# hzyu17/GaussianVI

Measured on AMD Instinct MI355X. Metric: sigma-point psi-evals/sec + NGD iters/sec, 1024-factor d=12 p=5 chain, higher is better.
Workload: dtype f64; 1 GPU; c3: T=1025 states, n=6; 1 step = 1 device-resident NGD iteration; restart every 30; factor_sets_columns=[K factors, d, GH degree p, N sigma points], factor_set_kinds=1024 x quadratic-prior d=12 p=5 (N=17217); 1025 x fixed-prior d=6 p=5 (N=1433), kernel_variant=6, chunks_per_factor=4, fused_pass=True, one_launch_factor_stage=False, mirror_pairs=False, fuse_trial=2

## Files before the change

### gaussianvi_amd/csrc/gvi_hip.hip

```cpp
#include "../../include/gvi_hip.h"

#include <hip/hip_runtime.h>
#include <hip/hip_ext.h>
#include <dlfcn.h>

#include <algorithm>
#include <chrono>
#include <cassert>
#include <cmath>
#include <cstdio>
#include <cstdlib>
#include <cstring>
#include <memory>
#include <map>
#include <set>
#include <string>
#include <thread>
#include <vector>

#include "host_linalg.hpp"
#include "kernels_bt.hpp"
#include "chain_launch.hpp"
#include "kernels_factor.hpp"
#include "kernels_orbit.hpp"
// ... 516 lines not shown
  }
  if (s.kind == KIND_QUAD_PRIOR) {
    switch (d) {
      case 2: launch_reg<2, PsiQuad<2, 1>>(a, grid, st); return true;
      case 4: launch_reg<4, PsiQuad<4, 2>>(a, grid, st); return true;
      case 6: launch_reg<6, PsiQuad<6, 3>>(a, grid, st); return true;
      case 8: launch_reg<8, PsiQuad<8, 4>>(a, grid, st); return true;
      case 12: launch_reg<12, PsiQuad<12, 6>>(a, grid, st); return true;
    }
  }
  if (s.kind == KIND_FIXED_PRIOR) {
    switch (d) {
      case 1: launch_reg<1, PsiQuad<1, 1>>(a, grid, st); return true;
      case 2: launch_reg<2, PsiQuad<2, 2>>(a, grid, st); return true;
      case 3: launch_reg<3, PsiQuad<3, 3>>(a, grid, st); return true;
      case 4: launch_reg<4, PsiQuad<4, 4>>(a, grid, st); return true;
      case 6: launch_reg<6, PsiQuad<6, 6>>(a, grid, st); return true;
      case 8: launch_reg<8, PsiQuad<8, 8>>(a, grid, st); return true;
      case 12: launch_reg<12, PsiQuad<12, 12>>(a, grid, st); return true;
    }
  }
  return false;
}

void dispatch_scost(gvi_ctx* c, const FactorSet& s, const MomArgs& a, int nchunk, hipStream_t st) {
  launch_scost<2>(s, a, nchunk, st);
}

bool orbit_supported(const gvi_ctx* c, const FactorSet& s) {
  if (!c->orbit || !(c->variant == 0 || c->variant == 6)) return false;
  if (s.kind != KIND_QUAD_PRIOR && s.kind != KIND_FIXED_PRIOR) return false;
  if (!(s.m == 2 || s.m == 6 || s.m == 12 || (s.m == 14 && s.table->orb.smax <= 4)) || s.d > 32) return false;
  if (s.m == 2 && s.table->orb.smax > 4) return false;
  const OrbitHost& o = s.table->orb;
  return o.ok && o.smax >= 1 && o.smax <= ORBIT_SMAX && !o.tile_s.empty();
}

gvi_status orbit_args(gvi_ctx* c, FactorSet& s, int full, OrbitArgs* out) {
  Table& t = *s.table;
  auto it = t.orb_bounds.find(s.nchunk);
  if (it == t.orb_bounds.end()) {
    const std::vector<int32_t> b = orbit_chunk_bounds(t.orb, s.nchunk);
    auto mem = std::make_unique<DevMem>();
    HIPCK(c, mem->ensure(b.size() * 4));
    HIPCK(c, hipMemcpy(mem->p, b.data(), b.size() * 4, hipMemcpyHostToDevice));
    it = t.orb_bounds.emplace(s.nchunk, std::move(mem)).first;
  }
  OrbitArgs a;
  a.H = s.H.d(); a.u0 = s.u0.d(); a.sgn = s.sgn.d(); a.partial = s.partial.d();
  a.K = s.K; a.d = s.d; a.nchunk = s.nchunk;
  a.pred = c->cur_pred; a.pred_val = c->cur_pred_val;
  const int waves = ((s.m == 6 && t.orb.smax <= 4) || s.m == 2) ? 4 : ((s.m == 12 && t.orb.smax <= 4) ? 3 : 2);
  const size_t lds_cap = std::min<size_t>(64 * 1024, 160 * 1024 / waves);
  a.copies = 1;
  while (a.copies * 2 <= c->orbit_copies && (size_t)4 * orbit_lds_doubles(s.d, s.m, a.copies * 2) * 8 <= lds_cap) a.copies *= 2;
  a.ob.cpk = (const uint64_t*)t.orb_cpk.p; a.ob.rpk = (const uint64_t*)t.orb_rpk.p; a.ob.mag = t.orb_mag.d(); a.ob.w = t.orb_w.d();
  a.ob.bounds = it->second->i();
  a.ob.norb_p = t.orb.norb_p; a.ob.w0 = t.orb.w0;
  {
    int32_t cum = 0;
    for (int sz = 7; sz >= 0; --sz) {
      if (sz >= 1 && sz <= t.orb.smax) cum += t.orb.cstride[sz] / 64;
      a.ob.cend[sz] = sz > t.orb.smax ? 0 : cum;
    }
    for (int sz = 0; sz < 8; ++sz) {
      const bool in = sz >= 1 && sz <= t.orb.smax;
      a.ob.cbase[sz] = in ? t.orb.cbase[sz] : 0;
      a.ob.cgrp[sz] = in ? t.orb.cgrp[sz] : 1;
      a.ob.cstride[sz] = in ? t.orb.cstride[sz] : 0;
    }
    a.ob.nb = 0;
    for (int i = 0; i < 5; ++i) a.ob.bnd[i] = 0;
    if (s.nchunk <= 4) {
      const std::vector<int32_t> b = orbit_chunk_bounds(t.orb, s.nchunk);
      a.ob.nb = s.nchunk;
      for (int i = 0; i <= s.nchunk; ++i) a.ob.bnd[i] = b[(size_t)i];
    }
  }
  (void)full;
  *out = a;
  return GVI_OK;
}

template <int M, int SMAX, int WAVES>
void launch_orbit_t(const OrbitArgs& a, bool full, bool all_pos, dim3 grid, size_t lds, hipStream_t st) {
  if (full && all_pos) hipLaunchKernelGGL((moments_orbit_kernel<M, SMAX, true, false, WAVES>), grid, dim3(256), lds, st, a);
  else if (full) hipLaunchKernelGGL((moments_orbit_kernel<M, SMAX, true, true, WAVES>), grid, dim3(256), lds, st, a);
  else if (all_pos) hipLaunchKernelGGL((moments_orbit_kernel<M, SMAX, false, false, WAVES>), grid, dim3(256), lds, st, a);
  else hipLaunchKernelGGL((moments_orbit_kernel<M, SMAX, false, true, WAVES>), grid, dim3(256), lds, st, a);
}

void launch_orbit(const OrbitArgs& a, int m, int smax, bool full, bool all_pos, hipStream_t st) {
  const dim3 grid((a.K + 3) / 4, a.nchunk);
  const size_t lds = (size_t)4 * orbit_lds_doubles(a.d, m, a.copies) * 8;
  if (m == 2) launch_orbit_t<2, 4, 4>(a, full, all_pos, grid, lds, st);
  else if (m == 14) launch_orbit_t<14, 4, 2>(a, full, all_pos, grid, lds, st);
  else if (m == 6 && smax <= 4) launch_orbit_t<6, 4, 4>(a, full, all_pos, grid, lds, st);
  else if (m == 6) launch_orbit_t<6, 6, 2>(a, full, all_pos, grid, lds, st);
  else if (smax <= 4) launch_orbit_t<12, 4, 3>(a, full, all_pos, grid, lds, st);
  else launch_orbit_t<12, 6, 2>(a, full, all_pos, grid, lds, st);
}

template <int M, int SMAX, int WAVES>
void launch_orbit_pair_t(const OrbitArgs& a0, const OrbitArgs& a1, bool full, size_t lds, hipStream_t st, hipEvent_t e0, hipEvent_t e1,
                         bool stack) {
  const int nbx0 = (a0.K + 3) / 4, nbx1 = (a1.K + 3) / 4;
  const int nb0 = nbx0 * a0.nchunk, nb1 = nbx1 * a1.nchunk;
  const int grid = stack ? std::max(nb0, nb1) : nb0 + nb1;
// ... 2840 lines not shown
```

### gaussianvi_amd/csrc/kernels_orbit.hpp

```cpp
#pragma once
#include <hip/hip_runtime.h>
#include <stdint.h>

#include "kernels_factor.hpp"

namespace gvi {

#ifdef GVI_FUSED_TIMING
__device__ unsigned long long* gvi_walk_stamps;
#endif

struct OrbitDev {
  const uint64_t* cpk;
  const uint64_t* rpk;
  const double* mag;
  const double* w;
  const int32_t* bounds;
  int64_t norb_p;
  double w0;
  int32_t cend[8];
  int32_t bnd[5];
  int32_t nb;
  int32_t cbase[8], cgrp[8], cstride[8];
};

template <int S>
struct OrbitRec { uint64_t cpk, rpk; double w; double mg[S]; };
template <typename T>
__device__ __forceinline__ T orbit_ld(const T* base, const uint32_t boff) { return *(const T*)((const char*)base + boff); }
template <int S>
__device__ __forceinline__ void orbit_load(const OrbitDev& ob, const uint32_t boff, OrbitRec<S>& r) {
  r.cpk = orbit_ld(ob.cpk, boff);
  if constexpr (S >= 1) r.rpk = orbit_ld(ob.rpk, boff);
  r.w = orbit_ld(ob.w, boff);
#pragma unroll
  for (int j = 0; j < S; ++j) r.mg[j] = orbit_ld(ob.mag + (size_t)j * ob.norb_p, boff);
}
struct OrbitNoPre { __device__ __forceinline__ void operator()() const {} };

template <int CTRL>
__device__ __forceinline__ double dpp_f64(const double v) {
  const int lo = __builtin_amdgcn_update_dpp(0, __double2loint(v), CTRL, 0xf, 0xf, false);
  const int hi = __builtin_amdgcn_update_dpp(0, __double2hiint(v), CTRL, 0xf, 0xf, false);
  return __hiloint2double(hi, lo);
}
__device__ __forceinline__ double wave_sum_f64(double v) {
  v += dpp_f64<0xB1>(v);
  v += dpp_f64<0x4E>(v);
  v += dpp_f64<0x124>(v);
  v += dpp_f64<0x128>(v);
  auto row = [&](int l) {
    return __hiloint2double(__builtin_amdgcn_readlane(__double2hiint(v), l), __builtin_amdgcn_readlane(__double2loint(v), l));
  };
  return (row(0) + row(16)) + (row(32) + row(48));
}

struct OrbitArgs {
  const double* H;
  const double* u0;
  const double* sgn;
  double* partial;
  int K, d, nchunk;
  int copies;
  const double* pred;
  double pred_val;
  OrbitDev ob;
};

__host__ __device__ constexpr int orbit_hstride(int M) { return M == 12 ? 14 : M; }

__device__ __forceinline__ void lds_add_f64(double* p, double v) {
  __hip_atomic_fetch_add(p, v, __ATOMIC_RELAXED, __HIP_MEMORY_SCOPE_WORKGROUP);
}
template <int S, typename Pre>
__device__ __forceinline__ void orbit_accumulate(const int sh, const int (&c)[S], const uint64_t rpk, const double (&mg)[S], const double wp,
                                                 const double E0, const double (&Eij)[S * (S - 1) / 2 + 1], const double (&Oi)[S],
                                                 double* accb, Pre&& pre) {
  constexpr int NV = 2 * S + S * (S - 1) / 2;
  const double w4 = wp + wp;
  double val[NV];
  {
    double mgl[S];
#pragma unroll
    for (int j = 0; j < S; ++j) { mgl[j] = mg[j]; asm volatile("" : "+v"(mgl[j]) : "v"(E0)); }
    int n = 0, e = 0;
#pragma unroll
    for (int i = 0; i < S; ++i) {
      const double wm = wp * mgl[i];
      val[n++] = w4 * mgl[i] * Oi[i];
      val[n++] = wm * mgl[i] * E0;
#pragma unroll
      for (int j = i + 1; j < S; ++j) val[n++] = wm * mgl[j] * Eij[e++];
    }
  }
  pre();
  char* const base = (char*)accb;
  char* const base1 = base + (1u << sh);
  unsigned A[S], B[S];
#pragma unroll
  for (int i = 0; i < S; ++i) {
    const unsigned lo = (unsigned)rpk, hi = (unsigned)(rpk >> 32);
    const unsigned R = i < 3 ? (lo >> (10 * i)) & 1023u : (hi >> (10 * (i - 3))) & 1023u;
    A[i] = R << sh;
    B[i] = (unsigned)c[i] << sh;
  }
  int n = 0;
#pragma unroll
  for (int i = 0; i < S; ++i) {
    lds_add_f64((double*)(base1 + B[i]), val[n]); ++n;
    lds_add_f64((double*)(base + (A[i] + B[i])), val[n]); ++n;
#pragma unroll
    for (int j = i + 1; j < S; ++j) { lds_add_f64((double*)(base + (A[i] + B[j])), val[n]); ++n; }
  }
}

template <int M, int S, bool FULL, bool SIGNED, typename Pre>
__device__ __forceinline__ void orbit_walk(const int lc, const uint64_t cpk, const uint64_t rpk, const double (&mg)[S], const double w,
                                           const double* Hl, double* accl, const double (&su0)[M], const double (&sg)[M],
                                           const double k0, double& m0, Pre&& pre) {
  int c[S];
#pragma unroll
  for (int j = 0; j < S; ++j) c[j] = (int)((cpk >> (8 * j)) & 255u);
  constexpr bool HREG = M * S <= 36 && !(M == 6 && S >= 4);
  constexpr int NH = 1 << (S - 1);
  double hcol[HREG ? S : 1][M];
  const double* hp[S];
#pragma unroll
  for (int j = 0; j < S; ++j) {
    hp[j] = Hl + c[j] * orbit_hstride(M);
    if constexpr (HREG) {
#pragma unroll
      for (int r = 0; r < M; ++r) hcol[j][r] = hp[j][r];
    }
  }
  int sig[S];
#pragma unroll
  for (int j = 0; j < S; ++j) sig[j] = j == S - 1 ? 1 : -1;
  double v[M];
#pragma unroll
  for (int r = 0; r < M; ++r) v[r] = mg[S - 1] * (HREG ? hcol[S - 1][r] : hp[S - 1][r]);
#pragma unroll
  for (int j = 0; j < S - 1; ++j) {
    if constexpr (!HREG) {
#pragma unroll
      for (int r = 0; r < M; ++r) asm volatile("" : "+v"(v[r]) :: "memory");
    }
#pragma unroll
    for (int r = 0; r < M; ++r) v[r] = fma(-mg[j], HREG ? hcol[j][r] : hp[j][r], v[r]);
  }
  constexpr bool H0REG = !HREG && M * (S + 9) <= 168;
  double h0[H0REG ? M : 1];
  if constexpr (H0REG) {
#pragma unroll
    for (int r = 0; r < M; ++r) h0[r] = hp[0][r];
  }
  constexpr bool WHT_BIG = M <= 6;
  constexpr bool WHT = FULL && S >= 2 && (S <= 4 || WHT_BIG);
  constexpr int LBMAX = S == 4 ? 2 : 3;
  constexpr int LB = S - 1 < LBMAX ? S - 1 : LBMAX;
  constexpr int BLK = 1 << LB;
  double cpv[WHT ? BLK : 1], lv[WHT ? BLK : 1];
  double E0 = 0.0, Eij[S * (S - 1) / 2 + 1], Oi[S];
#pragma unroll
  for (int e = 0; e < S * (S - 1) / 2 + 1; ++e) Eij[e] = 0.0;
#pragma unroll
  for (int j = 0; j < S; ++j) Oi[j] = 0.0;
#pragma unroll
  for (int g = 0; g < NH; ++g) {
    const int jn = g + 1 < NH ? __builtin_ctz(g + 1) : 0;
    double hn[M];
    if constexpr (!HREG) {
// ... 21 lines not shown
      if ((g & (BLK - 1)) == BLK - 1) {
#pragma unroll
        for (int j = 0; j < LB; ++j) {
#pragma unroll
          for (int bb = 0; bb < BLK; ++bb) {
            if (!(bb & (1 << j))) {
              const double c0v = cpv[bb], c1v = cpv[bb | (1 << j)], l0v = lv[bb], l1v = lv[bb | (1 << j)];
              cpv[bb] = c0v + c1v; cpv[bb | (1 << j)] = c1v - c0v;
              lv[bb] = l0v + l1v; lv[bb | (1 << j)] = l1v - l0v;
            }
          }
        }
        const bool first = g == BLK - 1;
        E0 = first ? cpv[0] : E0 + cpv[0];
        int e = 0;
#pragma unroll
        for (int i = 0; i < S; ++i) {
          {
            const double t = i < LB ? lv[1 << i] : lv[0];
            const bool pos = i < LB || sig[i] > 0;
            Oi[i] = first ? (pos ? t : -t) : (pos ? Oi[i] + t : Oi[i] - t);
          }
#pragma unroll
          for (int j = i + 1; j < S; ++j) {
            const double t = j < LB ? cpv[(1 << i) | (1 << j)] : (i < LB ? cpv[1 << i] : cpv[0]);
            const bool pos = (j < LB ? 1 : sig[j]) * (i < LB ? 1 : sig[i]) > 0;
            Eij[e] = first ? (pos ? t : -t) : (pos ? Eij[e] + t : Eij[e] - t);
            ++e;
          }
        }
      }
    } else {
      E0 += cp;
      if (FULL) {
        int e = 0;
#pragma unroll
        for (int i = 0; i < S; ++i) {
          Oi[i] = sig[i] > 0 ? Oi[i] + l : Oi[i] - l;
#pragma unroll
          for (int j = i + 1; j < S; ++j) { Eij[e] = sig[i] * sig[j] > 0 ? Eij[e] + cp : Eij[e] - cp; ++e; }
        }
      }
    }
    if (g + 1 < NH) {
      sig[jn] = -sig[jn];
      const double t2 = (sig[jn] > 0 ? 2.0 : -2.0) * mg[jn];
#pragma unroll
      for (int r = 0; r < M; ++r) v[r] = fma(t2, HREG ? hcol[jn][r] : ((H0REG && jn == 0) ? h0[r] : hn[r]), v[r]);
    }
  }
  const double wp = w + w;
  m0 = fma(wp, E0, m0);
  if constexpr (FULL) {
    orbit_accumulate<S>(lc + 3, c, rpk, mg, wp, E0, Eij, Oi, accl, pre);
  } else {
    pre();
  }
}

template <int S, bool SIGNED, typename Pre>
__device__ __forceinline__ void orbit_walk_split(const int lc, const uint64_t cpk, const uint64_t rpk, const double (&mg)[S], const double w,
                                                 const double* Hl, double* accl, const double (&su0)[12], const double (&sg)[12],
                                                 const double k0, double& m0, Pre&& pre) {
  constexpr int MH = 6, HS = orbit_hstride(12), NH = 1 << (S - 1), LB = 3, BLK = 8;
  static_assert(S >= 4 && S <= 6, "split walk: s = 4, 5, 6 (blocks of 8 Gray steps)");
  int c[S];
#pragma unroll
  for (int j = 0; j < S; ++j) c[j] = (int)((cpk >> (8 * j)) & 255u);
  double E0 = 0.0, Eij[S * (S - 1) / 2 + 1], Oi[S];
#pragma unroll
  for (int e = 0; e < S * (S - 1) / 2 + 1; ++e) Eij[e] = 0.0;
#pragma unroll
  for (int j = 0; j < S; ++j) Oi[j] = 0.0;
#pragma clang loop unroll(disable)
  for (int half = 0; half < 2; ++half) {
    double suh[MH], sgh[MH];
#pragma unroll
    for (int r = 0; r < MH; ++r) {
      suh[r] = half ? su0[MH + r] : su0[r];
      sgh[r] = SIGNED ? (half ? sg[MH + r] : sg[r]) : 1.0;
    }
    const double kk = half ? 0.0 : k0;
    double hcol[S][MH];
#pragma unroll
    for (int j = 0; j < S; ++j) {
      const double* hp = Hl + c[j] * HS + half * MH;
#pragma unroll
      for (int r = 0; r < MH; ++r) hcol[j][r] = hp[r];
    }
    int sig[S];
#pragma unroll
    for (int j = 0; j < S; ++j) sig[j] = j == S - 1 ? 1 : -1;
    double v[MH];
#pragma unroll
    for (int r = 0; r < MH; ++r) v[r] = mg[S - 1] * hcol[S - 1][r];
#pragma unroll
    for (int j = 0; j < S - 1; ++j) {
#pragma unroll
      for (int r = 0; r < MH; ++r) v[r] = fma(-mg[j], hcol[j][r], v[r]);
    }
    double cpv[BLK], lv[BLK];
#pragma unroll
    for (int g = 0; g < NH; ++g) {
      const int jn = g + 1 < NH ? __builtin_ctz(g + 1) : 0;
      double q = 0.0, l = 0.0;
#pragma unroll
      for (int r = 0; r < MH; ++r) {
        q = SIGNED ? fma(sgh[r] * v[r], v[r], q) : fma(v[r], v[r], q);
        l = fma(suh[r], v[r], l);
      }
      const double cp = q + kk;
      int b = 0;
#pragma unroll
      for (int j = 0; j < LB; ++j) b |= (sig[j] > 0 ? 1 : 0) << j;
      cpv[b] = cp;
      lv[b] = l;
      if ((g & (BLK - 1)) == BLK - 1) {
#pragma unroll
        for (int j = 0; j < LB; ++j) {
#pragma unroll
          for (int bb = 0; bb < BLK; ++bb) {
            if (!(bb & (1 << j))) {
              const double c0v = cpv[bb], c1v = cpv[bb | (1 << j)], l0v = lv[bb], l1v = lv[bb | (1 << j)];
              cpv[bb] = c0v + c1v; cpv[bb | (1 << j)] = c1v - c0v;
              lv[bb] = l0v + l1v; lv[bb | (1 << j)] = l1v - l0v;
            }
          }
        }
        E0 += cpv[0];
        int e = 0;
#pragma unroll
        for (int i = 0; i < S; ++i) {
          {
            const double t = i < LB ? lv[1 << i] : lv[0];
            const bool pos = i < LB || sig[i] > 0;
            Oi[i] = pos ? Oi[i] + t : Oi[i] - t;
          }
#pragma unroll
          for (int j = i + 1; j < S; ++j) {
            const double t = j < LB ? cpv[(1 << i) | (1 << j)] : (i < LB ? cpv[1 << i] : cpv[0]);
            const bool pos = (j < LB ? 1 : sig[j]) * (i < LB ? 1 : sig[i]) > 0;
            Eij[e] = pos ? Eij[e] + t : Eij[e] - t;
            ++e;
          }
        }
      }
      if (g + 1 < NH) {
        sig[jn] = -sig[jn];
        const double t2 = (sig[jn] > 0 ? 2.0 : -2.0) * mg[jn];
#pragma unroll
        for (int r = 0; r < MH; ++r) v[r] = fma(t2, hcol[jn][r], v[r]);
      }
    }
  }
  const double wp = w + w;
  m0 = fma(wp, E0, m0);
  orbit_accumulate<S>(lc + 3, c, rpk, mg, wp, E0, Eij, Oi, accl, pre);
}

template <int M, int S, bool FULL, bool SIGNED>
__device__ __forceinline__ void orbit_gray(const double (&hcol)[S][M], const double (&mg)[S], const double (&su0)[M], const double (&sg)[M],
                                           const double k0, double& E0, double (&Eij)[S * (S - 1) / 2 + 1], double (&Oi)[S]) {
  static_assert(S <= 3, "orbit_gray: one butterfly block");
  constexpr int NH = 1 << (S - 1), LB = S - 1, BLK = NH;
  constexpr bool WHT = FULL && S >= 2;
  int sig[S];
#pragma unroll
  for (int j = 0; j < S; ++j) sig[j] = j == S - 1 ? 1 : -1;
  double v[M];
#pragma unroll
  for (int r = 0; r < M; ++r) v[r] = mg[S - 1] * hcol[S - 1][r];
#pragma unroll
  for (int j = 0; j < S - 1; ++j) {
#pragma unroll
    for (int r = 0; r < M; ++r) v[r] = fma(-mg[j], hcol[j][r], v[r]);
  }
  double cpv[WHT ? BLK : 1], lv[WHT ? BLK : 1];
  E0 = 0.0;
#pragma unroll
  for (int e = 0; e < S * (S - 1) / 2 + 1; ++e) Eij[e] = 0.0;
#pragma unroll
  for (int j = 0; j < S; ++j) Oi[j] = 0.0;
#pragma unroll
  for (int g = 0; g < NH; ++g) {
    const int jn = g + 1 < NH ? __builtin_ctz(g + 1) : 0;
    double q = 0.0, l = 0.0;
#pragma unroll
    for (int r = 0; r < M; ++r) {
      q = SIGNED ? fma(sg[r] * v[r], v[r], q) : fma(v[r], v[r], q);
      if (FULL) l = fma(su0[r], v[r], l);
    }
    const double cp = q + k0;
    if constexpr (WHT) {
      int b = 0;
#pragma unroll
      for (int j = 0; j < LB; ++j) b |= (sig[j] > 0 ? 1 : 0) << j;
      cpv[b] = cp;
      lv[b] = l;
      if (g == NH - 1) {
#pragma unroll
        for (int j = 0; j < LB; ++j) {
#pragma unroll
          for (int bb = 0; bb < BLK; ++bb) {
            if (!(bb & (1 << j))) {
              const double c0v = cpv[bb], c1v = cpv[bb | (1 << j)], l0v = lv[bb], l1v = lv[bb | (1 << j)];
              cpv[bb] = c0v + c1v; cpv[bb | (1 << j)] = c1v - c0v;
              lv[bb] = l0v + l1v; lv[bb | (1 << j)] = l1v - l0v;
            }
          }
        }
        E0 = cpv[0];
        int e = 0;
#pragma unroll
        for (int i = 0; i < S; ++i) {
          Oi[i] = i < LB ? lv[1 << i] : lv[0];
#pragma unroll
          for (int j = i + 1; j < S; ++j) { Eij[e] = j < LB ? cpv[(1 << i) | (1 << j)] : cpv[1 << i]; ++e; }
        }
      }
    } else {
      E0 += cp;
      if (FULL) {
        int e = 0;
#pragma unroll
        for (int i = 0; i < S; ++i) {
          Oi[i] = sig[i] > 0 ? Oi[i] + l : Oi[i] - l;
#pragma unroll
          for (int j = i + 1; j < S; ++j) { Eij[e] = sig[i] * sig[j] > 0 ? Eij[e] + cp : Eij[e] - cp; ++e; }
        }
      }
    }
    if (g + 1 < NH) {
      sig[jn] = -sig[jn];
      const double t2 = (sig[jn] > 0 ? 2.0 : -2.0) * mg[jn];
#pragma unroll
      for (int r = 0; r < M; ++r) v[r] = fma(t2, hcol[jn][r], v[r]);
    }
  }
}

template <int S>
struct OrbitWm { double w; double mg[S]; };
template <int S>
__device__ __forceinline__ void orbit_load_wm(const OrbitDev& ob, const uint32_t boff, OrbitWm<S>& r) {
  r.w = orbit_ld(ob.w, boff);
#pragma unroll
  for (int j = 0; j < S; ++j) r.mg[j] = orbit_ld(ob.mag + (size_t)j * ob.norb_p, boff);
}

template <int M, int S, bool FULL, bool SIGNED>
__device__ __forceinline__ void orbit_class_grouped(const OrbitDev& ob, const int lc, const int t0, const int t1, const int tfirst,
                                                    const uint32_t lane8, const double* Hl, double* accl, const double (&su0)[M],
                                                    const double (&sg)[M], const double k0, double& m0) {
  static_assert(M * S <= 36, "support-major classes keep the support's columns in registers");
  constexpr int NV = 2 * S + S * (S - 1) / 2;
  const int G = ob.cgrp[S];
  const uint32_t gstride8 = (uint32_t)ob.cstride[S] * 8u;
  for (int t = t0; t < t1; ++t) {
    const uint32_t boff0 = ((uint32_t)ob.cbase[S] + (uint32_t)(t - tfirst) * 64u) * 8u + lane8;
    const uint64_t cpk = orbit_ld(ob.cpk, boff0), rpk = orbit_ld(ob.rpk, boff0);
    OrbitWm<S> cur;
    orbit_load_wm<S>(ob, boff0, cur);
    int c[S];
    double hcol[S][M];
#pragma unroll
    for (int j = 0; j < S; ++j) {
      c[j] = (int)((cpk >> (8 * j)) & 255u);
      const double* hp = Hl + c[j] * orbit_hstride(M);
#pragma unroll
      for (int r = 0; r < M; ++r) hcol[j][r] = hp[r];
    }
    double acc[FULL ? NV : 1];
#pragma unroll
    for (int q = 0; q < (FULL ? NV : 1); ++q) acc[q] = 0.0;
    for (int g = 0; g < G; ++g) {
      double mg[S];
#pragma unroll
      for (int j = 0; j < S; ++j) mg[j] = cur.mg[j];
      const double w = cur.w;
      double E0, Eij[S * (S - 1) / 2 + 1], Oi[S];
      orbit_gray<M, S, FULL, SIGNED>(hcol, mg, su0, sg, k0, E0, Eij, Oi);
      const uint32_t bn = boff0 + (uint32_t)(g + 1 < G ? g + 1 : g) * gstride8;
      __builtin_amdgcn_sched_barrier(0);
      orbit_load_wm<S>(ob, bn, cur);
      __builtin_amdgcn_sched_barrier(0);
      const double wp = w + w;
      m0 = fma(wp, E0, m0);
      if constexpr (FULL) {
        const double w4 = wp + wp;
        int n = 0, e = 0;
#pragma unroll
        for (int i = 0; i < S; ++i) {
          const double wm = wp * mg[i];
          acc[n] = fma(w4 * mg[i], Oi[i], acc[n]); ++n;
          acc[n] = fma(wm * mg[i], E0, acc[n]); ++n;
#pragma unroll
          for (int j = i + 1; j < S; ++j) { acc[n] = fma(wm * mg[j], Eij[e], acc[n]); ++n; ++e; }
        }
      }
    }
    if constexpr (FULL) {
      const int sh = lc + 3;
      char* const base = (char*)accl;
      char* const base1 = base + (1u << sh);
      unsigned A[S], B[S];
#pragma unroll
      for (int i = 0; i < S; ++i) {
        const unsigned R = ((unsigned)rpk >> (10 * i)) & 1023u;
        A[i] = R << sh;
        B[i] = (unsigned)c[i] << sh;
      }
      int n = 0;
#pragma unroll
      for (int i = 0; i < S; ++i) {
        lds_add_f64((double*)(base1 + B[i]), acc[n]); ++n;
        lds_add_f64((double*)(base + (A[i] + B[i])), acc[n]); ++n;
#pragma unroll
        for (int j = i + 1; j < S; ++j) { lds_add_f64((double*)(base + (A[i] + B[j])), acc[n]); ++n; }
      }
    }
  }
}

constexpr int ORBIT_GROUP_SMAX = 3;

template <int M, int S, bool FULL, bool SIGNED>
__device__ __forceinline__ void orbit_class(const OrbitDev& ob, const int lc, const int t0, const int t1, const int tfirst, const uint32_t lane8,
                                            const double* Hl, double* accl, const double (&su0)[M], const double (&sg)[M], const double k0,
                                            double& m0) {
  if (t0 >= t1) return;
  constexpr bool PIPE = S <= 3;
  OrbitRec<S> cur;
  const uint32_t cb8 = ((uint32_t)ob.cbase[S] - (uint32_t)tfirst * 64u) * 8u + lane8;
  if constexpr (PIPE) orbit_load<S>(ob, cb8 + (uint32_t)t0 * 512u, cur);
  for (int t = t0; t < t1; ++t) {
    if constexpr (!PIPE) orbit_load<S>(ob, cb8 + (uint32_t)t * 512u, cur);
    const int tn = t + 1 < t1 ? t + 1 : t;
    auto pre = [&]() {
      if constexpr (PIPE) {
        __builtin_amdgcn_sched_barrier(0);
        orbit_load<S>(ob, cb8 + (uint32_t)tn * 512u, cur);
        __builtin_amdgcn_sched_barrier(0);
      }
    };
    const uint64_t cpk = cur.cpk, rpk = cur.rpk;
    const double w = cur.w;
    double mg[S];
#pragma unroll
    for (int j = 0; j < S; ++j) mg[j] = cur.mg[j];
    if constexpr (M == 12 && S >= 4 && FULL) orbit_walk_split<S, SIGNED>(lc, cpk, rpk, mg, w, Hl, accl, su0, sg, k0, m0, pre);
    else orbit_walk<M, S, FULL, SIGNED>(lc, cpk, rpk, mg, w, Hl, accl, su0, sg, k0, m0, pre);
  }
}

template <int M, int SMAX, bool FULL, bool SIGNED, bool FRESH = false>
__device__ __forceinline__ void orbit_wave(const OrbitArgs& a, const int k, const int chunk, double* lds, double* out,
                                           const double* Hpre = nullptr, const double* u0pre = nullptr) {
  const OrbitDev& ob = a.ob;
  const int lane = threadIdx.x & 63, d = a.d;
#ifdef GVI_FUSED_TIMING
  const long long wt_start = clock64();
#endif
  const int NP = FULL ? (d + 1) * (d + 2) / 2 : 1;
  int tb, te;
  if (ob.nb) { tb = ob.bnd[chunk]; te = ob.bnd[chunk + 1]; }
  else { tb = ob.bounds[chunk]; te = ob.bounds[chunk + 1]; }
  tb = __builtin_amdgcn_readfirstlane(tb);
  te = __builtin_amdgcn_readfirstlane(te);
  const uint32_t lane8 = (uint32_t)lane * 8u;
  const double* Hl = Hpre ? Hpre : lds;
  const int C = a.copies, lc = __builtin_ctz((unsigned)C);
  double* accl = lds + d * orbit_hstride(M);
  if (!Hpre) {
    const double* Hg = a.H + (size_t)k * M * d;
    for (int e = lane; e < d * M; e += 64) lds[(e / M) * orbit_hstride(M) + e % M] = Hg[e];
  }
  if (FULL)
    for (int e = lane; e < NP * C; e += 64) accl[e] = 0.0;
  double* accme = accl + (lane & (C - 1));
  double su0[M], sg[M], k0 = 0.0;
#pragma unroll
  for (int r = 0; r < M; ++r) {
    double u;
    if (u0pre) {
      const double t = u0pre[r];
      u = __hiloint2double(__builtin_amdgcn_readfirstlane(__double2hiint(t)), __builtin_amdgcn_readfirstlane(__double2loint(t)));
    } else u = FRESH ? __builtin_nontemporal_load(a.u0 + (size_t)k * M + r) : a.u0[(size_t)k * M + r];
    sg[r] = SIGNED ? a.sgn[(size_t)k * M + r] : 1.0;
    su0[r] = SIGNED ? sg[r] * u : u;
    k0 = fma(su0[r], u, k0);
  }
  wave_lds_sync();
  double m0 = 0.0;
#ifdef GVI_FUSED_TIMING
  long long wt_last = clock64(), wt_acc[6] = {0, 0, 0, 0, 0, 0}, wt_n[5] = {0, 0, 0, 0, 0};
  wt_acc[0] = wt_last - wt_start;
#define ORBIT_CLASS_STAMP(S_, n_) do { if ((S_) <= 4) { const long long now = clock64(); wt_acc[S_] += now - wt_last; wt_n[S_] += (n_); wt_last = now; } } while (0)
#else
#define ORBIT_CLASS_STAMP(S_, n_) do { } while (0)
#endif
  int tcur = tb;
#define ORBIT_RUN_CLASS(S_)                                                                           \
  {                                                                                                   \
    const int e_ = te < ob.cend[S_] ? te : ob.cend[S_];                                                \
    if (tcur < e_) {                                                                                  \
      if constexpr (S_ <= ORBIT_GROUP_SMAX && M * S_ <= 36) orbit_class_grouped<M, S_, FULL, SIGNED>(ob, lc, tcur, e_, ob.cend[S_ + 1], lane8, Hl, accme, su0, sg, k0, m0); \
      else orbit_class<M, S_, FULL, SIGNED>(ob, lc, tcur, e_, ob.cend[S_ + 1], lane8, Hl, accme, su0, sg, k0, m0);            \
      ORBIT_CLASS_STAMP(S_, e_ - tcur); tcur = e_;                                                     \
    }                                                                                                 \
  }
  if constexpr (SMAX > 4) {
    ORBIT_RUN_CLASS(6)
    ORBIT_RUN_CLASS(5)
  }
  ORBIT_RUN_CLASS(4)
  ORBIT_RUN_CLASS(3)
  ORBIT_RUN_CLASS(2)
  ORBIT_RUN_CLASS(1)
#undef ORBIT_RUN_CLASS
#undef ORBIT_CLASS_STAMP
  m0 = wave_sum_f64(m0);
  if (chunk == 0) m0 = fma(ob.w0, k0, m0);
  wave_lds_sync();
  if (lane == 0) out[0] = m0;
  if (FULL) {
    if (C == 8) {
      for (int e = 1 + lane; e < NP; e += 64) {
        int rot = (lane >> 2) & 7;
        asm volatile("" : "+v"(rot));
        double c8[8];
#pragma unroll
        for (int q = 0; q < 8; ++q) c8[q] = accl[e * 8 + ((q + rot) & 7)];
        double t = c8[0];
#pragma unroll
        for (int q = 1; q < 8; ++q) t += c8[q];
        out[e] = t;
      }
    } else {
      for (int e = 1 + lane; e < NP; e += 64) {
        const int rot = (lane >> 2) & (C - 1);
        double t = accl[e * C + rot];
        for (int q = 1; q < C; ++q) t += accl[e * C + ((q + rot) & (C - 1))];
        out[e] = t;
      }
    }
  }
#ifdef GVI_FUSED_TIMING
  if (gvi_walk_stamps && lane == 0 && (blockIdx.x % 146) == 0) {
    wt_acc[5] = clock64() - wt_last;
    unsigned long long* ws = gvi_walk_stamps + (((blockIdx.x / 146) * 4 + (threadIdx.x >> 6)) * 2 + (d == 12 ? 0 : 1)) * 12;
    for (int i = 0; i < 6; ++i) ws[i] = (unsigned long long)wt_acc[i];
    for (int i = 1; i < 5; ++i) ws[6 + i] = (unsigned long long)wt_n[i];
  }
#endif
}

template <bool FULL>
__device__ __forceinline__ double* orbit_out(const OrbitArgs& a, const int k, const int chunk) {
  return a.partial + ((size_t)k * a.nchunk + chunk) * (FULL ? (a.d + 1) * (a.d + 2) / 2 : 1);
}

__host__ __device__ inline int orbit_lds_doubles(int d, int M, int copies) {
  return (d * orbit_hstride(M) + copies * (d + 1) * (d + 2) / 2 + 1) & ~1;
}

template <int M, int SMAX, bool FULL, bool SIGNED, int WAVES>
__global__ __launch_bounds__(256, WAVES) void moments_orbit_kernel(OrbitArgs a) {
  extern __shared__ double sm[];
  const int wave = __builtin_amdgcn_readfirstlane(threadIdx.x >> 6);
  const int k = (int)blockIdx.x * 4 + wave;
  if (pred_skip(a.pred, a.pred_val)) return;
  if (k >= a.K) return;
  orbit_wave<M, SMAX, FULL, SIGNED>(a, k, (int)blockIdx.y, sm + (size_t)wave * orbit_lds_doubles(a.d, M, a.copies),
                                    orbit_out<FULL>(a, k, (int)blockIdx.y));
}

template <int M, int SMAX, bool FULL, bool SIGNED, int WAVES>
__global__ __launch_bounds__(256, WAVES) void moments_orbit_pair_kernel(OrbitArgs a0, OrbitArgs a1, int nbx0, int nb0, int nbx1) {
  extern __shared__ double sm[];
  if (pred_skip(a0.pred, a0.pred_val)) return;
  const int wave = __builtin_amdgcn_readfirstlane(threadIdx.x >> 6);
  int id = (int)blockIdx.x;
  if (nbx1 < 0) {
    const int nx1 = -nbx1;
    const int l0 = orbit_lds_doubles(a0.d, M, a0.copies), l1 = orbit_lds_doubles(a1.d, M, a1.copies);
    double* mine = sm + (size_t)wave * (l0 > l1 ? l0 : l1);
    if (id < nb0) {
      const int k = (id % nbx0) * 4 + wave, chunk = id / nbx0;
      if (k < a0.K) orbit_wave<M, SMAX, FULL, SIGNED>(a0, k, chunk, mine, orbit_out<FULL>(a0, k, chunk));
    }
    const int k1 = (id % nx1) * 4 + wave, chunk1 = id / nx1;
    if (chunk1 < a1.nchunk && k1 < a1.K) orbit_wave<M, SMAX, FULL, SIGNED>(a1, k1, chunk1, mine, orbit_out<FULL>(a1, k1, chunk1));
    return;
  }
  const bool second = id >= nb0;
  if (second) id -= nb0;
  const int nbx = second ? nbx1 : nbx0;
  const int k = (id % nbx) * 4 + wave, chunk = id / nbx;
  if (!second) {
    if (k < a0.K) orbit_wave<M, SMAX, FULL, SIGNED>(a0, k, chunk, sm + (size_t)wave * orbit_lds_doubles(a0.d, M, a0.copies), orbit_out<FULL>(a0, k, chunk));
  } else {
    if (k < a1.K) orbit_wave<M, SMAX, FULL, SIGNED>(a1, k, chunk, sm + (size_t)wave * orbit_lds_doubles(a1.d, M, a1.copies), orbit_out<FULL>(a1, k, chunk));
  }
}

}
```

### gaussianvi_amd/csrc/orbits.hpp

```cpp
#pragma once
#include <algorithm>
#include <cstdint>
#include <cstring>
#include <unordered_map>
#include <vector>

namespace gvi {

constexpr int ORBIT_SMAX = 6;

struct OrbitHost {
  bool ok = false;
  int smax = 0;
  double w0 = 0.0;
  int64_t count[ORBIT_SMAX + 1] = {0};
  int64_t norb_p = 0;
  std::vector<uint64_t> cpk;
  std::vector<uint64_t> rpk;
  std::vector<double> mag;
  std::vector<double> w;
  std::vector<int32_t> tile_s, tile_first, tile_g, tile_gstride;
  int32_t cbase[ORBIT_SMAX + 2] = {0}, cgrp[ORBIT_SMAX + 2] = {0}, cstride[ORBIT_SMAX + 2] = {0};
};

inline double orbit_tile_cost(int s, int g) {
  static const double walk[ORBIT_SMAX + 1] = {0, 300, 800, 1300, 2500, 5200, 10800};
  return g * walk[s] + 600.0;
}

inline OrbitHost build_orbits(int d, int64_t N, const double* Z, const double* w, bool verify, int group_smax = 3) {
  OrbitHost o;
  if (d > 32) return o;
  struct Rep { int64_t row; int s; };
  std::vector<Rep> reps;
  int64_t covered = 0;
  bool have_origin = false;
  for (int64_t i = 0; i < N; ++i) {
    const double* z = Z + (size_t)i * d;
    int s = 0;
    bool pos = true;
    for (int a = 0; a < d; ++a) {
      if (z[a] != 0.0) { ++s; pos = pos && z[a] > 0.0; }
    }
    if (!pos) continue;
    if (s > ORBIT_SMAX) return o;
    if (s == 0) { have_origin = true; o.w0 = w[i]; covered += 1; continue; }
    reps.push_back({i, s});
    covered += (int64_t)1 << s;
  }
  if (covered != N) return o;
  if (verify) {
    auto hash_row = [&](const double* z) {
      uint64_t h = 1469598103934665603ull;
      for (int a = 0; a < d; ++a) {
        double v = z[a] < 0 ? -z[a] : z[a];
        if (v == 0.0) v = 0.0;
        uint64_t b;
        std::memcpy(&b, &v, 8);
        h = (h ^ b) * 1099511628211ull;
      }
      return h;
    };
    std::unordered_map<uint64_t, int64_t> by_key;
    by_key.reserve(reps.size() * 2);
    for (const Rep& r : reps) by_key.emplace(hash_row(Z + (size_t)r.row * d), r.row);
    for (int64_t i = 0; i < N; ++i) {
      const double* z = Z + (size_t)i * d;
      bool zero = true;
      for (int a = 0; a < d; ++a) zero = zero && z[a] == 0.0;
      if (zero) continue;
      auto it = by_key.find(hash_row(z));
      if (it == by_key.end()) return o;
      const double* zr = Z + (size_t)it->second * d;
      for (int a = 0; a < d; ++a)
        if ((z[a] < 0 ? -z[a] : z[a]) != zr[a]) return o;
      if (w[i] != w[it->second]) return o;
    }
  }
  (void)have_origin;
  std::stable_sort(reps.begin(), reps.end(), [](const Rep& a, const Rep& b) { return a.s > b.s; });
// ... 42 lines not shown
          for (int part = 0; part < best_f; ++part) cp.slots.emplace_back(gr.begin() + (size_t)part * cp.g, gr.begin() + (size_t)(part + 1) * cp.g);
      } else {
        cp.g = 1;
        for (size_t i = 0; i < cnt; ++i) cp.slots.push_back({(int64_t)(ri + i)});
      }
      ri += cnt;
    }
  }
  o.norb_p = 0;
  for (int s = o.smax; s >= 1; --s) o.norb_p += (int64_t)plan[s].g * (int64_t)((plan[s].slots.size() + 63) / 64 * 64);
  o.cpk.assign(o.norb_p, 0);
  o.rpk.assign(o.norb_p, 0);
  o.mag.assign((size_t)o.smax * o.norb_p, 0.0);
  o.w.assign(o.norb_p, 0.0);
  int64_t pos = 0;
  for (int s = o.smax; s >= 1; --s) {
    const ClassPlan& cp = plan[s];
    const int64_t cnt = (int64_t)cp.slots.size(), padded = (cnt + 63) / 64 * 64;
    o.cbase[s] = (int32_t)pos; o.cgrp[s] = cp.g; o.cstride[s] = (int32_t)padded;
    for (int64_t t = 0; t < padded / 64; ++t) {
      o.tile_s.push_back(s); o.tile_first.push_back((int32_t)(pos + t * 64));
      o.tile_g.push_back(cp.g); o.tile_gstride.push_back((int32_t)padded);
    }
    int64_t P = 1;
    if (cnt > 64) {
      P = cnt / 64 + 1;
      auto gcd = [](int64_t a, int64_t b) { while (b) { const int64_t t = a % b; a = b; b = t; } return a; };
      while (gcd(P, cnt) != 1) ++P;
    }
    for (int64_t q = 0; q < cnt; ++q) {
      const std::vector<int64_t>& slot = cp.slots[(size_t)((q * P) % cnt)];
      for (int g = 0; g < cp.g; ++g) {
        const Rep& rep = reps[(size_t)slot[(size_t)g]];
        const double* z = Z + (size_t)rep.row * d;
        const int64_t e = pos + (int64_t)g * padded + q;
        uint64_t pk = 0, rk = 0;
        int j = 0;
        for (int a = 0; a < d; ++a)
          if (z[a] != 0.0) {
            pk |= (uint64_t)a << (8 * j);
            const uint64_t R = (uint64_t)(1 + d + a * d - a * (a - 1) / 2 - a);
            rk |= R << (j < 3 ? 10 * j : 32 + 10 * (j - 3));
            o.mag[(size_t)j * o.norb_p + e] = z[a];
            ++j;
          }
        o.cpk[e] = pk;
        o.rpk[e] = rk;
        o.w[e] = w[rep.row];
      }
    }
    pos += (int64_t)cp.g * padded;
  }
  if (o.norb_p >= ((int64_t)1 << 28)) return OrbitHost();
  o.ok = true;
  return o;
}

inline std::vector<int32_t> orbit_chunk_bounds(const OrbitHost& o, int nchunk) {
  const int nt = (int)o.tile_s.size();
  std::vector<double> cost(nt);
  double total = 0.0, biggest = 0.0;
  for (int t = 0; t < nt; ++t) { cost[t] = orbit_tile_cost(o.tile_s[t], o.tile_g[t]); total += cost[t]; biggest = std::max(biggest, cost[t]); }
  auto fill = [&](double cap, std::vector<int32_t>* out) {
    int t = 0, used = 0;
    if (out) out->assign((size_t)nchunk + 1, nt);
    if (out) (*out)[0] = 0;
    while (t < nt) {
      if (used == nchunk) return false;
      double sum = 0.0;
      while (t < nt && sum + cost[t] <= cap * (1.0 + 1e-12)) sum += cost[t++];
      ++used;
      if (out) (*out)[(size_t)used] = t;
    }
    return true;
  };
  double lo = std::max(biggest, total / std::max(nchunk, 1)), hi = std::max(total, biggest);
  for (int it = 0; it < 60 && hi - lo > 1e-9 * hi; ++it) {
    const double mid = 0.5 * (lo + hi);
    if (fill(mid, nullptr)) hi = mid; else lo = mid;
  }
  std::vector<int32_t> b;
  fill(hi, &b);
  return b;
}

}
```

Before: 209.5 billion psi-evals/s.

## Split orbit LDS accumulator into hot diagonal and off-diagonal copies with host-assigned copy slots

Splits the per-wave LDS accumulator into a 'hot' region for linear and diagonal terms with many replicated copies and an off-diagonal region with fewer copies, cutting LDS footprint. Each orbit gets a copy index chosen on the host by a greedy search that tries to minimise same-address and bank collisions among lanes in each 16-lane group. The index is packed into the top bits of cpk, replacing the old lane-based copy choice. The aim is to reduce LDS atomic contention and bank conflicts, at the cost of a more complex final reduction and extra host build time.

```diff
diff --git a/gaussianvi_amd/csrc/gvi_hip.hip b/gaussianvi_amd/csrc/gvi_hip.hip
--- a/gaussianvi_amd/csrc/gvi_hip.hip
+++ b/gaussianvi_amd/csrc/gvi_hip.hip
@@ -592,8 +592,9 @@
   a.pred = c->cur_pred; a.pred_val = c->cur_pred_val;
   const int waves = ((s.m == 6 && t.orb.smax <= 4) || s.m == 2) ? 4 : ((s.m == 12 && t.orb.smax <= 4) ? 3 : 2);
   const size_t lds_cap = std::min<size_t>(64 * 1024, 160 * 1024 / waves);
+  const int want = s.m == 12 ? c->orbit_copies : std::min(16, 2 * c->orbit_copies);
   a.copies = 1;
-  while (a.copies * 2 <= c->orbit_copies && (size_t)4 * orbit_lds_doubles(s.d, s.m, a.copies * 2) * 8 <= lds_cap) a.copies *= 2;
+  while (a.copies * 2 <= want && (size_t)4 * orbit_lds_doubles(s.d, s.m, a.copies * 2) * 8 <= lds_cap) a.copies *= 2;
   a.ob.cpk = (const uint64_t*)t.orb_cpk.p; a.ob.rpk = (const uint64_t*)t.orb_rpk.p; a.ob.mag = t.orb_mag.d(); a.ob.w = t.orb_w.d();
   a.ob.bounds = it->second->i();
   a.ob.norb_p = t.orb.norb_p; a.ob.w0 = t.orb.w0;
diff --git a/gaussianvi_amd/csrc/kernels_orbit.hpp b/gaussianvi_amd/csrc/kernels_orbit.hpp
--- a/gaussianvi_amd/csrc/kernels_orbit.hpp
+++ b/gaussianvi_amd/csrc/kernels_orbit.hpp
@@ -72,10 +72,46 @@
 __device__ __forceinline__ void lds_add_f64(double* p, double v) {
   __hip_atomic_fetch_add(p, v, __ATOMIC_RELAXED, __HIP_MEMORY_SCOPE_WORKGROUP);
 }
+
+__host__ __device__ constexpr int orbit_off_copies(int M, int copies) { return M == 12 ? copies : (copies >= 8 ? copies / 4 : 1); }
+
+struct OrbitAcc {
+  char* hot;
+  char* off;
+  int shh, sho;
+  unsigned mh, mo;
+};
+template <int S, int NV>
+__device__ __forceinline__ void orbit_add_all(const OrbitAcc& L, const uint64_t cpk, const int (&c)[S], const uint64_t rpk, const double (&val)[NV]) {
+  const unsigned k = (unsigned)(cpk >> 32) >> 24;
+  char* const hb = L.hot + ((k & L.mh) << 3);
+  char* const ob = L.off + ((k & L.mo) << 3);
+  const unsigned hstep = 1u << L.shh;
+  unsigned X[S], A[S], B[S];
+#pragma unroll
+  for (int i = 0; i < S; ++i) {
+    const unsigned lo = (unsigned)rpk, hi = (unsigned)(rpk >> 32);
+    const unsigned R = i < 3 ? (lo >> (10 * i)) & 1023u : (hi >> (10 * (i - 3))) & 1023u;
+    X[i] = (unsigned)c[i] << (L.shh + 1);
+    B[i] = (unsigned)c[i] << L.sho;
+    A[i] = (R << L.sho) - B[i];
+  }
+  int n = 0;
+#pragma unroll
+  for (int i = 0; i < S; ++i) {
+    char* const hp = hb + X[i];
+    lds_add_f64((double*)hp, val[n]); ++n;
+    lds_add_f64((double*)(hp + hstep), val[n]); ++n;
+    char* const op = ob + A[i];
+#pragma unroll
+    for (int j = i + 1; j < S; ++j) { lds_add_f64((double*)(op + B[j]), val[n]); ++n; }
+  }
+}
+
 template <int S, typename Pre>
-__device__ __forceinline__ void orbit_accumulate(const int sh, const int (&c)[S], const uint64_t rpk, const double (&mg)[S], const double wp,
-                                                 const double E0, const double (&Eij)[S * (S - 1) / 2 + 1], const double (&Oi)[S],
-                                                 double* accb, Pre&& pre) {
+__device__ __forceinline__ void orbit_accumulate(const OrbitAcc& L, const uint64_t cpk, const int (&c)[S], const uint64_t rpk, const double (&mg)[S],
+                                                 const double wp, const double E0, const double (&Eij)[S * (S - 1) / 2 + 1], const double (&Oi)[S],
+                                                 Pre&& pre) {
   constexpr int NV = 2 * S + S * (S - 1) / 2;
   const double w4 = wp + wp;
   double val[NV];
@@ -94,29 +130,12 @@
     }
   }
   pre();
-  char* const base = (char*)accb;
-  char* const base1 = base + (1u << sh);
-  unsigned A[S], B[S];
-#pragma unroll
-  for (int i = 0; i < S; ++i) {
-    const unsigned lo = (unsigned)rpk, hi = (unsigned)(rpk >> 32);
-    const unsigned R = i < 3 ? (lo >> (10 * i)) & 1023u : (hi >> (10 * (i - 3))) & 1023u;
-    A[i] = R << sh;
-    B[i] = (unsigned)c[i] << sh;
-  }
-  int n = 0;
-#pragma unroll
-  for (int i = 0; i < S; ++i) {
-    lds_add_f64((double*)(base1 + B[i]), val[n]); ++n;
-    lds_add_f64((double*)(base + (A[i] + B[i])), val[n]); ++n;
-#pragma unroll
-    for (int j = i + 1; j < S; ++j) { lds_add_f64((double*)(base + (A[i] + B[j])), val[n]); ++n; }
-  }
+  orbit_add_all<S>(L, cpk, c, rpk, val);
 }
 
 template <int M, int S, bool FULL, bool SIGNED, typename Pre>
-__device__ __forceinline__ void orbit_walk(const int lc, const uint64_t cpk, const uint64_t rpk, const double (&mg)[S], const double w,
-                                           const double* Hl, double* accl, const double (&su0)[M], const double (&sg)[M],
+__device__ __forceinline__ void orbit_walk(const OrbitAcc& L, const uint64_t cpk, const uint64_t rpk, const double (&mg)[S], const double w,
+                                           const double* Hl, const double (&su0)[M], const double (&sg)[M],
                                            const double k0, double& m0, Pre&& pre) {
   int c[S];
 #pragma unroll
@@ -244,15 +263,15 @@
   const double wp = w + w;
   m0 = fma(wp, E0, m0);
   if constexpr (FULL) {
-    orbit_accumulate<S>(lc + 3, c, rpk, mg, wp, E0, Eij, Oi, accl, pre);
+    orbit_accumulate<S>(L, cpk, c, rpk, mg, wp, E0, Eij, Oi, pre);
   } else {
     pre();
   }
 }
 
 template <int S, bool SIGNED, typename Pre>
-__device__ __forceinline__ void orbit_walk_split(const int lc, const uint64_t cpk, const uint64_t rpk, const double (&mg)[S], const double w,
-                                                 const double* Hl, double* accl, const double (&su0)[12], const double (&sg)[12],
+__device__ __forceinline__ void orbit_walk_split(const OrbitAcc& L, const uint64_t cpk, const uint64_t rpk, const double (&mg)[S], const double w,
+                                                 const double* Hl, const double (&su0)[12], const double (&sg)[12],
                                                  const double k0, double& m0, Pre&& pre) {
   constexpr int MH = 6, HS = orbit_hstride(12), NH = 1 << (S - 1), LB = 3, BLK = 8;
   static_assert(S >= 4 && S <= 6, "split walk: s = 4, 5, 6 (blocks of 8 Gray steps)");
@@ -347,7 +366,7 @@
   }
   const double wp = w + w;
   m0 = fma(wp, E0, m0);
-  orbit_accumulate<S>(lc + 3, c, rpk, mg, wp, E0, Eij, Oi, accl, pre);
+  orbit_accumulate<S>(L, cpk, c, rpk, mg, wp, E0, Eij, Oi, pre);
 }
 
 template <int M, int S, bool FULL, bool SIGNED>
@@ -441,8 +460,8 @@
 }
 
 template <int M, int S, bool FULL, bool SIGNED>
-__device__ __forceinline__ void orbit_class_grouped(const OrbitDev& ob, const int lc, const int t0, const int t1, const int tfirst,
-                                                    const uint32_t lane8, const double* Hl, double* accl, const double (&su0)[M],
+__device__ __forceinline__ void orbit_class_grouped(const OrbitDev& ob, const OrbitAcc& L, const int t0, const int t1, const int tfirst,
+                                                    const uint32_t lane8, const double* Hl, const double (&su0)[M],
                                                     const double (&sg)[M], const double k0, double& m0) {
   static_assert(M * S <= 36, "support-major classes keep the support's columns in registers");
   constexpr int NV = 2 * S + S * (S - 1) / 2;
@@ -491,34 +510,15 @@
         }
       }
     }
-    if constexpr (FULL) {
-      const int sh = lc + 3;
-      char* const base = (char*)accl;
-      char* const base1 = base + (1u << sh);
-      unsigned A[S], B[S];
-#pragma unroll
-      for (int i = 0; i < S; ++i) {
-        const unsigned R = ((unsigned)rpk >> (10 * i)) & 1023u;
-        A[i] = R << sh;
-        B[i] = (unsigned)c[i] << sh;
-      }
-      int n = 0;
-#pragma unroll
-      for (int i = 0; i < S; ++i) {
-        lds_add_f64((double*)(base1 + B[i]), acc[n]); ++n;
-        lds_add_f64((double*)(base + (A[i] + B[i])), acc[n]); ++n;
-#pragma unroll
-        for (int j = i + 1; j < S; ++j) { lds_add_f64((double*)(base + (A[i] + B[j])), acc[n]); ++n; }
-      }
-    }
+    if constexpr (FULL) orbit_add_all<S>(L, cpk, c, rpk, acc);
   }
 }
 
 constexpr int ORBIT_GROUP_SMAX = 3;
 
 template <int M, int S, bool FULL, bool SIGNED>
-__device__ __forceinline__ void orbit_class(const OrbitDev& ob, const int lc, const int t0, const int t1, const int tfirst, const uint32_t lane8,
-                                            const double* Hl, double* accl, const double (&su0)[M], const double (&sg)[M], const double k0,
+__device__ __forceinline__ void orbit_class(const OrbitDev& ob, const OrbitAcc& L, const int t0, const int t1, const int tfirst, const uint32_t lane8,
+                                            const double* Hl, const double (&su0)[M], const double (&sg)[M], const double k0,
                                             double& m0) {
   if (t0 >= t1) return;
   constexpr bool PIPE = S <= 3;
@@ -540,8 +540,30 @@
     double mg[S];
 #pragma unroll
     for (int j = 0; j < S; ++j) mg[j] = cur.mg[j];
-    if constexpr (M == 12 && S >= 4 && FULL) orbit_walk_split<S, SIGNED>(lc, cpk, rpk, mg, w, Hl, accl, su0, sg, k0, m0, pre);
-    else orbit_walk<M, S, FULL, SIGNED>(lc, cpk, rpk, mg, w, Hl, accl, su0, sg, k0, m0, pre);
+    if constexpr (M == 12 && S >= 4 && FULL) orbit_walk_split<S, SIGNED>(L, cpk, rpk, mg, w, Hl, su0, sg, k0, m0, pre);
+    else orbit_walk<M, S, FULL, SIGNED>(L, cpk, rpk, mg, w, Hl, su0, sg, k0, m0, pre);
+  }
+}
+
+template <int C>
+__device__ __forceinline__ double orbit_copy_sum_c(const double* p, const int lane) {
+  int rot = (lane >> (4 - __builtin_ctz((unsigned)C))) & (C - 1);
+  asm volatile("" : "+v"(rot));
+  double v[C];
+#pragma unroll
+  for (int q = 0; q < C; ++q) v[q] = p[(q + rot) & (C - 1)];
+  double t = v[0];
+#pragma unroll
+  for (int q = 1; q < C; ++q) t += v[q];
+  return t;
+}
+__device__ __forceinline__ double orbit_copy_sum(const double* p, const int C, const int lane) {
+  switch (C) {
+    case 16: return orbit_copy_sum_c<16>(p, lane);
+    case 8: return orbit_copy_sum_c<8>(p, lane);
+    case 4: return orbit_copy_sum_c<4>(p, lane);
+    case 2: return orbit_copy_sum_c<2>(p, lane);
+    default: return p[0];
   }
 }
 
@@ -561,15 +583,23 @@
   te = __builtin_amdgcn_readfirstlane(te);
   const uint32_t lane8 = (uint32_t)lane * 8u;
   const double* Hl = Hpre ? Hpre : lds;
-  const int C = a.copies, lc = __builtin_ctz((unsigned)C);
-  double* accl = lds + d * orbit_hstride(M);
+  const int CH = a.copies, CO = orbit_off_copies(M, CH);
+  const int NO = d * (d - 1) / 2;
+  double* const hot = lds + d * orbit_hstride(M);
+  double* const offr = hot + 2 * d * CH;
+  OrbitAcc L;
+  L.shh = __builtin_ctz((unsigned)CH) + 3;
+  L.sho = __builtin_ctz((unsigned)CO) + 3;
+  L.mh = (unsigned)CH - 1u;
+  L.mo = (unsigned)CO - 1u;
+  L.hot = (char*)hot;
+  L.off = (char*)offr - ((unsigned)(d + 2) << L.sho);
   if (!Hpre) {
     const double* Hg = a.H + (size_t)k * M * d;
     for (int e = lane; e < d * M; e += 64) lds[(e / M) * orbit_hstride(M) + e % M] = Hg[e];
   }
   if (FULL)
-    for (int e = lane; e < NP * C; e += 64) accl[e] = 0.0;
-  double* accme = accl + (lane & (C - 1));
+    for (int e = lane; e < 2 * d * CH + NO * CO; e += 64) hot[e] = 0.0;
   double su0[M], sg[M], k0 = 0.0;
 #pragma unroll
   for (int r = 0; r < M; ++r) {
@@ -596,8 +626,8 @@
   {                                                                                                   \
     const int e_ = te < ob.cend[S_] ? te : ob.cend[S_];                                                \
     if (tcur < e_) {                                                                                  \
-      if constexpr (S_ <= ORBIT_GROUP_SMAX && M * S_ <= 36) orbit_class_grouped<M, S_, FULL, SIGNED>(ob, lc, tcur, e_, ob.cend[S_ + 1], lane8, Hl, accme, su0, sg, k0, m0); \
-      else orbit_class<M, S_, FULL, SIGNED>(ob, lc, tcur, e_, ob.cend[S_ + 1], lane8, Hl, accme, su0, sg, k0, m0);            \
+      if constexpr (S_ <= ORBIT_GROUP_SMAX && M * S_ <= 36) orbit_class_grouped<M, S_, FULL, SIGNED>(ob, L, tcur, e_, ob.cend[S_ + 1], lane8, Hl, su0, sg, k0, m0); \
+      else orbit_class<M, S_, FULL, SIGNED>(ob, L, tcur, e_, ob.cend[S_ + 1], lane8, Hl, su0, sg, k0, m0);                     \
       ORBIT_CLASS_STAMP(S_, e_ - tcur); tcur = e_;                                                     \
     }                                                                                                 \
   }
@@ -616,25 +646,14 @@
   wave_lds_sync();
   if (lane == 0) out[0] = m0;
   if (FULL) {
-    if (C == 8) {
-      for (int e = 1 + lane; e < NP; e += 64) {
-        int rot = (lane >> 2) & 7;
-        asm volatile("" : "+v"(rot));
-        double c8[8];
-#pragma unroll
-        for (int q = 0; q < 8; ++q) c8[q] = accl[e * 8 + ((q + rot) & 7)];
-        double t = c8[0];
-#pragma unroll
-        for (int q = 1; q < 8; ++q) t += c8[q];
-        out[e] = t;
-      }
-    } else {
-      for (int e = 1 + lane; e < NP; e += 64) {
-        const int rot = (lane >> 2) & (C - 1);
-        double t = accl[e * C + rot];
-        for (int q = 1; q < C; ++q) t += accl[e * C + ((q + rot) & (C - 1))];
-        out[e] = t;
-      }
+    for (int h = lane; h < 2 * d; h += 64) {
+      const int c = h >> 1;
+      out[(h & 1) ? 1 + d + c * d - c * (c - 1) / 2 : 1 + c] = orbit_copy_sum(hot + h * CH, CH, lane);
+    }
+    for (int p = lane; p < NO; p += 64) {
+      int r = 0, q = p;
+      while (q >= d - 1 - r) { q -= d - 1 - r; ++r; }
+      out[p + d + 2 + r] = orbit_copy_sum(offr + p * CO, CO, lane);
     }
   }
 #ifdef GVI_FUSED_TIMING
@@ -653,7 +672,7 @@
 }
 
 __host__ __device__ inline int orbit_lds_doubles(int d, int M, int copies) {
-  return (d * orbit_hstride(M) + copies * (d + 1) * (d + 2) / 2 + 1) & ~1;
+  return (d * orbit_hstride(M) + 2 * d * copies + d * (d - 1) / 2 * orbit_off_copies(M, copies) + 1) & ~1;
 }
 
 template <int M, int SMAX, bool FULL, bool SIGNED, int WAVES>
diff --git a/gaussianvi_amd/csrc/orbits.hpp b/gaussianvi_amd/csrc/orbits.hpp
--- a/gaussianvi_amd/csrc/orbits.hpp
+++ b/gaussianvi_amd/csrc/orbits.hpp
@@ -26,6 +26,98 @@
 inline double orbit_tile_cost(int s, int g) {
   static const double walk[ORBIT_SMAX + 1] = {0, 300, 800, 1300, 2500, 5200, 10800};
   return g * walk[s] + 600.0;
+}
+
+constexpr int ORBIT_COPY_SHIFT = 56;
+inline int orbit_copy_index(uint64_t cpk) { return (int)((cpk >> ORBIT_COPY_SHIFT) & 15u); }
+
+inline void orbit_add_offsets(int d, int s, const int* c, bool padding, int k, int ch, int co, int64_t* out) {
+  const int64_t off = (int64_t)2 * d * ch * 8, kh = (int64_t)(k & (ch - 1)) * 8, ko = (int64_t)(k & (co - 1)) * 8;
+  int n = 0;
+  for (int i = 0; i < s; ++i) {
+    const int64_t ci = padding ? 0 : c[i];
+    out[n++] = ci * 2 * ch * 8 + kh;
+    out[n++] = (ci * 2 + 1) * ch * 8 + kh;
+    for (int j = i + 1; j < s; ++j) {
+      const int64_t R = padding ? 0 : 1 + d + (int64_t)c[i] * d - (int64_t)c[i] * (c[i] - 1) / 2 - c[i];
+      const int64_t cj = padding ? 0 : c[j];
+      out[n++] = off + (R - ci + cj - (d + 2)) * co * 8 + ko;
+    }
+  }
+}
+
+struct OrbitAddCost { int64_t same = 0, bank = 0; };
+inline OrbitAddCost orbit_add_cost(const int64_t* addr ) {
+  OrbitAddCost r;
+  for (int a = 0; a < 64; ++a) {
+    bool seen = false, seen_in_group = false, bank_taken = false;
+    for (int b = 0; b < a; ++b) {
+      const bool group = (a >> 4) == (b >> 4);
+      if (addr[b] == addr[a]) { seen = true; seen_in_group = seen_in_group || group; }
+      else if (group && ((addr[b] >> 3) & 15) == ((addr[a] >> 3) & 15)) bank_taken = true;
+    }
+    if (seen) ++r.same;
+    if (bank_taken && !seen_in_group) ++r.bank;
+  }
+  return r;
+}
+
+inline void orbit_assign_copies(OrbitHost& o, int d) {
+  constexpr int CH = 16, CO = 4, NADD = 2 * ORBIT_SMAX + ORBIT_SMAX * (ORBIT_SMAX - 1) / 2;
+  const int nt = (int)o.tile_s.size();
+  const size_t span = (size_t)2 * d * CH + (size_t)d * (d - 1) / 2 * CO + 1;
+  std::vector<int> cnt(span * NADD, 0), gcnt(span * NADD, 0);
+  for (int t = 0; t < nt; ++t) {
+    const int s = o.tile_s[t], nadd = 2 * s + s * (s - 1) / 2;
+    int c[64][ORBIT_SMAX];
+    bool pad[64];
+    for (int lane = 0; lane < 64; ++lane) {
+      const int64_t q = (int64_t)o.tile_first[t] + lane;
+      pad[lane] = o.w[q] == 0.0 && o.rpk[q] == 0;
+      for (int j = 0; j < s; ++j) c[lane][j] = (int)((o.cpk[q] >> (8 * j)) & 255u);
+    }
+    int64_t ad[64][NADD];
+    int kbest[64];
+    for (int g = 0; g < 4; ++g) {
+      bool used[CH] = {false};
+      int64_t bank[NADD][16];
+      for (int n = 0; n < nadd; ++n)
+        for (int b = 0; b < 16; ++b) bank[n][b] = -1;
+      for (int lane = 16 * g; lane < 16 * g + 16; ++lane) {
+        int64_t best = -1;
+        int bk = 0;
+        for (int k = 0; k < CH; ++k) {
+          if (used[k]) continue;
+          int64_t a[NADD];
+          orbit_add_offsets(d, s, c[lane], pad[lane], k, CH, CO, a);
+          int64_t cost = 0;
+          for (int n = 0; n < nadd; ++n) {
+            const size_t i = (size_t)(a[n] >> 3) * NADD + n;
+            cost += 3 * cnt[i];
+            if (gcnt[i] == 0 && bank[n][(a[n] >> 3) & 15] >= 0) cost += 1;
+          }
+          if (best < 0 || cost < best) { best = cost; bk = k; }
+        }
+        used[bk] = true;
+        kbest[lane] = bk;
+        orbit_add_offsets(d, s, c[lane], pad[lane], bk, CH, CO, ad[lane]);
+        for (int n = 0; n < nadd; ++n) {
+          const size_t i = (size_t)(ad[lane][n] >> 3) * NADD + n;
+          cnt[i]++; gcnt[i]++;
+          bank[n][(ad[lane][n] >> 3) & 15] = ad[lane][n];
+        }
+      }
+      for (int lane = 16 * g; lane < 16 * g + 16; ++lane)
+        for (int n = 0; n < nadd; ++n) gcnt[(size_t)(ad[lane][n] >> 3) * NADD + n] = 0;
+    }
+    for (int lane = 0; lane < 64; ++lane) {
+      for (int n = 0; n < nadd; ++n) cnt[(size_t)(ad[lane][n] >> 3) * NADD + n] = 0;
+      for (int gi = 0; gi < o.tile_g[t]; ++gi) {
+        uint64_t& pk = o.cpk[(size_t)o.tile_first[t] + lane + (size_t)gi * o.tile_gstride[t]];
+        pk = (pk & ~((uint64_t)15 << ORBIT_COPY_SHIFT)) | ((uint64_t)kbest[lane] << ORBIT_COPY_SHIFT);
+      }
+    }
+  }
 }
 
 inline OrbitHost build_orbits(int d, int64_t N, const double* Z, const double* w, bool verify, int group_smax = 3) {
@@ -174,6 +266,7 @@
     pos += (int64_t)cp.g * padded;
   }
   if (o.norb_p >= ((int64_t)1 << 28)) return OrbitHost();
+  orbit_assign_copies(o, d);
   o.ok = true;
   return o;
 }
```

After: 204.8 billion psi-evals/s (median of 2 runs). 0.977x the previous value.
